# JuanTarrio/rebvo

Measured on NVIDIA H100. Metric: frames/sec @752x480 EuRoC replay (synthetic stand-in), detect+track+map; pose ATE vs reference in `parity`, higher is better.
Workload: dtype f32 scale space/detector + f64 tracker/EKF

## Files before the change

### include/rebvo_b200.h

```cpp
#ifndef REBVO_B200_H
#define REBVO_B200_H

#include <stdint.h>

#ifdef __cplusplus
extern "C" {
#endif

typedef struct rb_ctx rb_ctx;
typedef struct rb_map rb_map;
typedef struct rb_pipeline rb_pipeline;

enum rb_status {
    RB_OK = 0,
    RB_ERR_CUDA = -1,
    RB_ERR_ARG = -2,
    RB_ERR_NO_DEVICE = -3,
    RB_ERR_STATE = -4
};

typedef struct rb_keyline {
    int32_t p_inx;
    float m_m[2], u_m[2], n_m, score, c_p[2];
    int32_t _pad0;
// ... 72 lines not shown

int rb_map_create(rb_ctx *c, rb_map **out);
void rb_map_destroy(rb_map *m);
int rb_map_clone(const rb_map *src, rb_map **out);

int rb_map_upload_rgb(rb_map *m, const uint8_t *rgb);
int rb_map_upload_mono(rb_map *m, const uint8_t *mono);
int rb_map_upload_gray(rb_map *m, const float *gray);
int rb_map_dog_build(rb_map *m);
int rb_map_get_plane(rb_map *m, int which, float *out);
int rb_map_detect(rb_map *m, const rb_detect_params *p, double *tresh, int *l_kl_num, int *kn_out);
int rb_map_detect_ss(rb_map *m, rb_map *ss, const rb_detect_params *p, double *tresh, int *l_kl_num,
                     int *kn_out);
int rb_map_reestimate_thresh(rb_map *m, int knum, int nbins, float *out_thresh);
int rb_map_knum(rb_map *m, int *kn);
int rb_map_sync_host_keylines(rb_map *m, rb_keyline *dst, int capacity, int *kn);
int rb_map_load_keylines(rb_map *m, const rb_keyline *src, int kn, const int32_t *mask);
int rb_map_get_mask(rb_map *m, int32_t *out);

int rb_map_quantile(rb_map *m, double s_rho_min, double s_rho_max, double percentile, int nbins,
                    double *out);
int rb_map_build_field(rb_map *m, int radius, float min_mod);
int rb_map_get_field(rb_map *m, int32_t *out);
int rb_try_vel_rot(rb_map *fmap, rb_map *old, const double X[6], int reweight, int procjf,
                   double match_thresh, double s_rho_min, uint32_t match_num_thresh, double k_huber,
                   const double *res_in, double *res_out, double JtJ[36], double JtF[6], double *score);
int rb_minimizer_rv(rb_map *fmap, rb_map *old, double V[3], double W[3], double RVel[9], double RW0[9],
                    double match_thresh, int iter_max, int init_type, double reweight_distance,
                    double *rel_error, double *rel_error_score, double max_s_rho,
                    uint32_t match_num_thresh, int init_iter, double W_X[36], double *score);
// ... 69 lines not shown
```

### rebvo_b200/capi.py

```python
import ctypes as C
import os

import numpy as np

HERE = os.path.dirname(os.path.abspath(__file__))
LIB_PATH = os.environ.get("REBVO_B200_LIB") or os.path.join(HERE, "librebvo_b200.so")


class RbError(RuntimeError):
    pass


class Camera(C.Structure):
    _fields_ = [("w", C.c_int32), ("h", C.c_int32), ("ppx", C.c_float), ("ppy", C.c_float),
                ("zfx", C.c_float), ("zfy", C.c_float)]


class DetectParams(C.Structure):
    _fields_ = [("plane_fit_size", C.c_int32), ("pos_neg_thresh", C.c_double), ("dog_thresh", C.c_double),
                ("kl_max", C.c_int32), ("kl_ref", C.c_int32), ("gain", C.c_double),
                ("thresh_max", C.c_double), ("thresh_min", C.c_double)]


class Params(C.Structure):
# ... 36 lines not shown
KEYLINE = np.dtype({
    "names": ["p_inx", "m_m", "u_m", "n_m", "score", "c_p", "rho", "s_rho", "rho_nr", "s_rho_nr",
              "rho0", "s_rho0", "p_m", "p_m_0", "m_id", "m_id_f", "m_id_kf", "m_num", "m_m0", "n_m0",
              "p_id", "n_id", "net_id", "stereo_m_id", "stereo_rho", "stereo_s_rho"],
    "formats": ["i4", ("f4", 2), ("f4", 2), "f4", "f4", ("f4", 2), "f8", "f8", "f8", "f8", "f8", "f8",
                ("f4", 2), ("f4", 2), "i4", "i4", "i4", "i4", ("f4", 2), "f8", "i4", "i4", "i4", "i4",
                "f8", "f8"],
    "offsets": [0, 4, 12, 20, 24, 28, 40, 48, 56, 64, 72, 80, 88, 96, 104, 108, 112, 116, 120, 128,
                136, 140, 144, 148, 152, 160],
    "itemsize": 168})

SYMBOLS = ["rb_ctx_create", "rb_ctx_destroy", "rb_last_error", "rb_ctx_sync", "rb_ctx_box_plan",
           "rb_ctx_launch_count", "rb_map_create", "rb_map_destroy", "rb_map_clone", "rb_map_upload_rgb", "rb_map_upload_mono",
           "rb_map_upload_gray",
           "rb_map_dog_build", "rb_map_get_plane", "rb_map_detect", "rb_map_detect_ss", "rb_map_reestimate_thresh", "rb_map_knum",
           "rb_map_sync_host_keylines", "rb_map_load_keylines", "rb_map_get_mask", "rb_map_quantile",
           "rb_map_build_field", "rb_map_get_field", "rb_try_vel_rot", "rb_minimizer_rv", "rb_forward_match",
           "rb_map_rotate_keylines", "rb_directed_matching", "rb_map_regularize", "rb_map_ekf_update",
           "rb_map_rescale_opt", "rb_map_set_frame_count", "rb_pipeline_create", "rb_pipeline_destroy",
           "rb_pipeline_last_error", "rb_pipeline_push", "rb_pipeline_push_dev", "rb_pipeline_push_mono",
           "rb_pipeline_push_mono_dev", "rb_pipeline_reset",
           "rb_pipeline_map", "rb_pipeline_launch_count", "rb_pipeline_stage_ms", "rb_pipeline_stream",
           "rb_pipeline_event_record", "rb_pipeline_event_elapsed", "rb_pipeline_event_elapsed_between", "rb_pipeline_bench_pass",
           "rb_pipeline_set_imu", "rb_pipeline_set_mirror", "rb_pipeline_mirror", "rb_pipeline_set_undistort",
           "rb_pipeline_stage_profile",
           "rb_undistort_create", "rb_undistort_destroy", "rb_undistort_rgb", "rb_undistort_rgb_dev",
           "rb_try_vel", "rb_minimizer_v", "rb_ext_rot_vel", "rb_bias_correct", "rb_map_pack_net_keylines",
           "rb_nav_format_trajectory", "rb_nav_format_log", "rb_map_scale_space_path"]

_lib = None
# ... 176 lines not shown
    def detect(self, det, tresh, l_kl_num):
        t, l, kn = C.c_double(tresh), C.c_int(l_kl_num), C.c_int(0)
        self.ctx.check(self.L.rb_map_detect(self.h_, C.byref(det), C.byref(t), C.byref(l), C.byref(kn)))
        return kn.value, t.value, l.value

    def reestimate(self, knum, nbins):
        o = C.c_float(0)
        self.ctx.check(self.L.rb_map_reestimate_thresh(self.h_, knum, nbins, C.byref(o)))
        return o.value

    def knum(self):
        k = C.c_int(0)
        self.ctx.check(self.L.rb_map_knum(self.h_, C.byref(k)))
        return k.value

    def keylines(self):
        kn = self.knum()
        out = np.zeros(max(kn, 1), KEYLINE)
        k = C.c_int(0)
        self.ctx.check(self.L.rb_map_sync_host_keylines(self.h_, _p(out), len(out), C.byref(k)))
        return out[:kn]

    def scale_space_path(self):
        return int(self.L.rb_map_scale_space_path(self.h_))

    def pack_net(self, k_prof=1.0, capacity=None):
        cap = capacity if capacity is not None else max(self.knum(), 1)
        out = np.zeros((cap, 15), np.uint8)
        k = C.c_int(0)
        self.ctx.check(self.L.rb_map_pack_net_keylines(self.h_, C.c_double(k_prof), _p(out), cap, C.byref(k)))
# ... 255 lines not shown
```

### rebvo_b200/csrc/capi.cu

```cuda
#include <math.h>
#include <stdlib.h>
#include <new>

#include "common.cuh"
#include "tracker.cuh"

int rb_detect_upload_pinv(rb_ctx *c);

static void box_plan_one(double sigma, int box_n, int *box_d, double *sigma_r) {
    const double wideal = sqrt(12 * sigma * sigma / box_n + 1);
    int wl = (int)wideal;
    const int tmp = wl / 2;
    if (tmp * 2 == wl) wl--;
    const int m = (int)round((3 * box_n + 4 * box_n * wl + box_n * wl * wl - 12 * sigma * sigma) / (4 + 4 * wl));
    int i = 0;
    for (; i < m && i < box_n; i++) box_d[i] = wl;
    for (; i < box_n; i++) box_d[i] = wl + 2;
    *sigma_r = sqrt((m * wl * wl + (box_n - m) * (wl + 2.0) * (wl + 2.0) - box_n) / 12.0);
}

static void plane_fit_pinv(double pinv[3][25]) {
    const int ws = 2;
    double Phi[25][3];
    int k = 0;
// ... 491 lines not shown
    if ((r = read_state(m, &s))) return r;
    if (out_thresh) *out_thresh = s.retuned;
    return RB_OK;
}

extern "C" int rb_map_knum(rb_map *m, int *kn) {
    if (!m) return RB_ERR_ARG;
    RB_ENTER(m->c);
    MapState s;
    int r = read_state(m, &s);
    if (r) return r;
    *kn = s.kn;
    return RB_OK;
}

extern "C" int rb_map_scale_space_path(const rb_map *m) {
    if (!m || !m->ws.gray) return 0;
    return (m->ws.tma_row_ok ? 1 : 0) | (m->ws.tma_ok ? 2 : 0);
}

extern "C" int rb_map_sync_host_keylines(rb_map *m, rb_keyline *dst, int capacity, int *kn) {
    if (!m) return RB_ERR_ARG;
    RB_ENTER(m->c);
    rb_ctx *c = m->c;
    MapState s;
    int r = read_state(m, &s);
    if (r) return r;
    if (kn) *kn = s.kn;
    if (s.kn == 0) return RB_OK;
    if (!dst || capacity < s.kn) return RB_ERR_ARG;
// ... 53 lines not shown
```

### rebvo_b200/csrc/min_cluster.cuh

```cuda
#ifndef MC_T
#error "define MC_T and MC_NS before including min_cluster.cuh"
#endif
#undef MC_NW
#undef MC_MAXJ
#undef MC_NV
#define MC_NW (MC_T / 32)
#define MC_MAXJ (3584 / MC_T)
#define MC_NV (MC_MAXJ * MC_NW)

#ifndef MC_COMMON_PART
#define MC_COMMON_PART
#define MC_C 16
#define MC_GMAX 8
#define MC_PW 30
#define MC_XW 60
#ifndef MC_KPC_FAST
#define MC_KPC_FAST 1280
#endif
#define MC_SPIN_LIMIT (1ll << 29)
#define MC_BYTES_PER_KL 57

#ifdef RB_TVR_PROF
#define MC_STAMP(e, k) do { if (threadIdx.x == 0 && blockIdx.x < 16) g_tvr_prof[(blockIdx.x * 16 + (e)) * 16 + (k)] = clock64(); } while (0)
#else
// ... 454 lines not shown
    so3_exp(wz, RMf);
    sm.req[p][12] = RMf[0];
    sm.req[p][13] = RMf[1];
    sm.req[p][14] = RMf[3];
    sm.req[p][15] = RMf[4];
}

template <int XCHG>
__global__ void __cluster_dims__(MC_C, 1, 1) __launch_bounds__(MC_T, 1)
    k_minimizer_cluster(KLSoA old, const MapState *__restrict__ old_st, const unsigned long long *__restrict__ field,
                        const float4 *__restrict__ fpack, MapState *f_st, LMState *lm_out, int *abort_out, CamC cam,
                        McPlan plan, MinSetup su, FrameState *post_fs, FmBest *fm_best, int kpc_cap, ResPtrs gres,
                        unsigned long long *ll, MinCtl *ctl) {
    MC_STAMP(15, 0);
    const bool early = su.early_operands != 0 && su.a.match_num_thresh <= 255u;
    if (!early) {
        pdl_wait();
        pdl_launch();
    }
    MC_STAMP(15, 1);
    extern __shared__ __align__(16) unsigned char mc_dyn[];
    __shared__ McSmem sm;
    const int tid = threadIdx.x, lane = tid & 31, wid = tid >> 5;
    const int rank = (int)mc_cluster_rank();
    const int G = (int)(gridDim.x / MC_C), cl = (int)(blockIdx.x / MC_C);
    const bool first_cta = blockIdx.x == 0;
    const unsigned int seq0 = G > 1 ? __ldcg(&ctl->gen) : 0u;
    const int K0 = old_st->kn;
    if (K0 <= 0) {
        if (early) {
            pdl_wait();
            pdl_launch();
        }
        if (first_cta && tid == 0) {
// ... 45 lines not shown
        if (li < v.S) {
            const KlOp o = load_klop(old, v.base + li, cam);
            v.x0[li] = o.x0;
            v.y0[li] = o.y0;
            v.z0[li] = o.z0;
            v.s_rho[li] = o.s_rho;
            const unsigned int mn = (unsigned int)o.m_num;
            v.flag[li] = early ? (unsigned char)(mn < 255u ? mn : 255u) : (unsigned char)(mn < tc.mnt ? 1 : 0);
            v.res[0][li] = 0.0;
        } else {
            v.gres[0][v.base + li] = 0.0;
        }
    }
    if (early) {
        pdl_wait();
        pdl_launch();
        tc.s_rho_min = su.s_rho_from_state ? old_st->s_rho_q : su.max_s_rho;
        const unsigned int fc = su.fc_from_state ? f_st->frame_count : su.frame_count;
        tc.mnt = su.a.match_num_thresh < fc ? su.a.match_num_thresh : fc;
        const int ns = v.cnt < v.S ? v.cnt : v.S;
        for (int li = tid; li < ns; li += MC_T) v.flag[li] = (unsigned int)v.flag[li] < tc.mnt ? 1 : 0;
    }
    const bool fused = plan.merge_round >= 0;
    if (tid == 0) {
        sm.abort = su.debug_abort;
        lm_begin(sm.lm, old_st, f_st, su.VW, su.a, su.max_r, su.max_s_rho, su.s_rho_from_state, su.frame_count,
                 su.fc_from_state);
        if (fused) {
            for (int i = 0; i < 3; i++) {
                sm.lm.X[i] = sm.lm.Vel_in[i];
                sm.lm.X[3 + i] = sm.lm.W0_in[i];
// ... 17 lines not shown
    mc_cluster_sync();
    MC_STAMP(15, 2);

    for (int e = 0; e < plan.n; e++) {
        const int sa = plan.sa[e], sb = plan.sb[e];
        const bool two = sa != STEP_NONE;
        const bool RW = sb >= STEP_MAIN_FIRST;
        const bool PJ = !(sb == STEP_INIT_LAST_ZERO || sb == STEP_INIT_LAST_PRIOR);
        const int par = e & 1;
        const unsigned int nval = two ? 2 * MC_PW : MC_PW;
        const bool last = e == plan.n - 1;
        const bool merge = e == plan.merge_round;
        const bool next_two = !last && plan.sa[e + 1] != STEP_NONE;
        const int res_out_p[2] = {sm.req_res[0][1], sm.req_res[1][1]};
        MC_STAMP(e, 0);
        if (RW) mc_eval_pose<true, true>(sm, v, 0, old, tc, cam, field, fpack, last, tid, lane, wid);
        else if (PJ) mc_eval_pose<false, true>(sm, v, 0, old, tc, cam, field, fpack, last, tid, lane, wid);
        else mc_eval_pose<false, false>(sm, v, 0, old, tc, cam, field, fpack, last, tid, lane, wid);
        if (two) {
            if (PJ) mc_eval_pose<false, true>(sm, v, 1, old, tc, cam, field, fpack, false, tid, lane, wid);
            else mc_eval_pose<false, false>(sm, v, 1, old, tc, cam, field, fpack, false, tid, lane, wid);
        }
        __syncthreads();
        MC_STAMP(e, 1);
        const unsigned int seq = seq0 + 1u + (unsigned int)e;
        if (XCHG && tid == 0) mc_mbar_expect_tx(&sm.mbar[par], nval * MC_C * 8u);
        if (wid < 2 && (wid == 0 || two)) {
            const int p = wid;
            double t = lane < MC_PW ? sm.xout[p * MC_PW + lane] : 0.0;
            if (G > 1) {
// ... 194 lines not shown
```

### rebvo_b200/csrc/pipeline.cu

```cuda
#include <math.h>
#include <stdlib.h>
#include <new>

#include "common.cuh"
#include "lm.cuh"
#include "tracker.cuh"
#include "frame.cuh"

int rb_map_alloc(rb_ctx *c, rb_map **out, bool with_ws);

#define RB_NMAPS 3

#ifdef RB_TVR_PROF
__device__ unsigned long long g_trace[8192];
__device__ unsigned int g_trace_n;
__global__ void k_trace_mark(int tag) {
    unsigned long long t;
    asm volatile("mov.u64 %0, %globaltimer;" : "=l"(t));
    const unsigned int k = atomicAdd(&g_trace_n, 1u);
    if (k < 8192) g_trace[k] = ((unsigned long long)tag << 56) | (t & 0x00FFFFFFFFFFFFFFull);
}
extern "C" int rb_debug_fetch_trace(unsigned long long *out, unsigned int *n) {
    cudaMemcpyFromSymbol(n, g_trace_n, sizeof(unsigned int));
    cudaMemcpyFromSymbol(out, g_trace, sizeof(unsigned long long) * 8192);
// ... 7 lines not shown

struct ImuFlow;
struct rb_pipeline {
    rb_ctx *c;
    ImuFlow *imu;
    rb_params p;
    int max_batch;
    DogWS ws;
    rb_map *maps[RB_NMAPS];
    cudaStream_t det_stream;
    cudaEvent_t ev_dog, *ev_det, *ev_trk;
    bool overlap;
    bool q_fold;
    int ss_sub;
    bool map_fused;
    cudaStream_t resc_stream;
    cudaEvent_t ev_rfork, ev_rjoin;
    bool resc_open;
    cudaStream_t copy_stream;
    cudaEvent_t *ev_copy;
    const void **rgb_src_dev;
    const void **rgb_src_pin;
    int sub;
    DetChain *chain;
    FrameState *fs;
    rb_nav *nav_dev;
    rb_nav *nav_pin;
    int *abort_pin;
    uint8_t *rgb_pin;
    long long n_pushed;
// ... 170 lines not shown
    const char *ng = getenv("REBVO_B200_NO_GRAPH");
    pl->use_graph = !(ng && ng[0] == '1');
    const char *sp = getenv("REBVO_B200_STAGE_PROF");
    pl->prof_on = sp && sp[0] == '1';
    if (pl->prof_on) {
        pl->use_graph = false;
        pl->pcap = max_batch * 12 + 8;
        pl->pev = new (std::nothrow) cudaEvent_t[pl->pcap];
        pl->ptag = new (std::nothrow) int[pl->pcap];
        if (!pl->pev || !pl->ptag) return RB_ERR_ARG;
        for (int i = 0; i < pl->pcap; i++) RB_CUDA(cudaEventCreate(&pl->pev[i]));
    }
    {
        const char *mf = getenv("REBVO_B200_MAP_FUSED");
        pl->map_fused = mf ? atoi(mf) != 0 : false;
        const char *ov = getenv("REBVO_B200_OVERLAP");
        pl->overlap = !(ov && ov[0] == '0') && !pl->prof_on;
        pl->q_fold = getenv("REBVO_B200_Q_FOLD") && atoi(getenv("REBVO_B200_Q_FOLD")) != 0 && p->QCutOffNumBins >= 1 &&
                     p->QCutOffNumBins <= 128;
        pl->ss_sub = getenv("REBVO_B200_SS_SUB") ? atoi(getenv("REBVO_B200_SS_SUB")) : 0;
        if (pl->ss_sub < 4) pl->ss_sub = 0;
        pl->ev_det = new (std::nothrow) cudaEvent_t[max_batch];
        pl->ev_trk = new (std::nothrow) cudaEvent_t[max_batch];
        if (!pl->ev_det || !pl->ev_trk) return RB_ERR_ARG;
        memset(pl->ev_det, 0, sizeof(cudaEvent_t) * max_batch);
        memset(pl->ev_trk, 0, sizeof(cudaEvent_t) * max_batch);
        RB_CUDA(cudaStreamCreateWithFlags(&pl->det_stream, cudaStreamNonBlocking));
        RB_CUDA(cudaStreamCreateWithFlags(&pl->copy_stream, cudaStreamNonBlocking));
        const char *sb = getenv("REBVO_B200_SUB");
        pl->sub = sb ? atoi(sb) : 8;
// ... 156 lines not shown
    a.reweight_distance = p.ReweigthDistance;
    a.match_num_thresh = p.MatchNumThresh;
    RB_TRACE(c->stream, 2);
    bool folded = false;
    c->min_early = !pl->q_fold && (getenv("REBVO_B200_MIN_EARLY") ? atoi(getenv("REBVO_B200_MIN_EARLY")) != 0 : true);
    r = rb_minimizer_enqueue(c, neu, old, pl->fs->VW, &a, 0.0, true, 0, true, pl->fs, &folded);
    c->min_early = false;
    if (r) return r;
    RB_TRACE(c->stream, 3);
    prof_mark(pl, ST_MINIM);
    if (!folded) {
        k_frame_post_min<<<1, 1, 0, c->stream>>>(pl->fs, neu->ts);
        RB_LAUNCH_CHECK();
        if ((r = rb_forward_match_argmax_enqueue(c, old, neu))) return r;
    }
    if ((r = resc_join(pl))) return r;
    if ((r = rb_forward_match_apply_enqueue(c, old, neu, pl->fs->R0))) return r;
    RB_TRACE(c->stream, 11);
    prof_mark(pl, ST_FWD_ROT);
    if ((r = rb_directed_matching_enqueue(c, neu, old, &pl->fs->dm, p.MatchThreshModule, p.MatchThreshAngle,
                                          (double)p.SearchRange, p.LocationUncertaintyMatch, &pl->fs->do_match)))
        return r;
    RB_TRACE(c->stream, 4);
    prof_mark(pl, ST_DMATCH);
    const bool side = pl->resc_stream != nullptr && pl->mirror_on != 1;
    if (!pl->map_fused)
        if ((r = rb_regularize_ekf_enqueue(c, neu, p.RegularizeThresh, pl->fs, p.MatchThreshold, pl->fs->V,
                                           p.ReshapeQAbsolute, p.LocationUncertainty, &pl->fs->do_map,
                                           side ? old->st : nullptr, side ? nav_slot : nullptr, fa)))
            return r;
    RB_TRACE(c->stream, 9);
    prof_mark(pl, ST_REG_EKF);
    if (side) {
        cudaStream_t main_stream = c->stream;
        RB_CUDA(cudaEventRecord(pl->ev_rfork, main_stream));
        RB_CUDA(cudaStreamWaitEvent(pl->resc_stream, pl->ev_rfork, 0));
        c->stream = pl->resc_stream;
        r = rb_rescale_enqueue(c, neu, RB_RHO_MAX, 1, 0, &neu->st->do_map, nav_slot);
        c->stream = main_stream;
        if (r) return r;
        RB_CUDA(cudaEventRecord(pl->ev_rjoin, pl->resc_stream));
        pl->resc_open = true;
        RB_TRACE(c->stream, 5);
        return RB_OK;
    }
// ... 380 lines not shown
```

### rebvo_b200/csrc/tracker.cu

```cuda
#include "tracker.cuh"
#include "lm.cuh"
#include "frame.cuh"

#define TVR_T 256
#define RES_SENTINEL 0x7FF8DEADBEEF0001ull

#ifdef RB_TVR_PROF
__device__ long long g_tvr_prof[256 * 16];
#define TVR_STAMP(k) do { if (threadIdx.x == 0) g_tvr_prof[blockIdx.x * 16 + (k)] = clock64(); } while (0)
__device__ __forceinline__ long long tvr_gtime() {
    long long t;
    asm volatile("mov.u64 %0, %globaltimer;" : "=l"(t));
    return t;
}
#define TVR_GSTAMP(k) do { if (threadIdx.x == 0) g_tvr_prof[blockIdx.x * 16 + (k)] = tvr_gtime(); } while (0)
extern "C" int rb_debug_fetch(long long *out) {
    return (int)cudaMemcpyFromSymbol(out, g_tvr_prof, sizeof(long long) * 256 * 16);
}
#else
#define TVR_STAMP(k) do { } while (0)
#define TVR_GSTAMP(k) do { } while (0)
#endif

struct CamC {
// ... 1220 lines not shown
}

int rb_try_vel_rot_enqueue(rb_ctx *c, rb_map *fmap, rb_map *old, const double *X_dev, int reweight, int procjf,
                           double match_thresh, double s_rho_min, unsigned int mnt, unsigned int fc,
                           double k_huber) {
    if (fmap->field_radius <= 0) return RB_ERR_STATE;
    k_lm_single<<<1, 1, 0, c->stream>>>(fmap->ts, X_dev, 0, 1, (double)fmap->field_radius, match_thresh, s_rho_min,
                                        mnt, fc, k_huber);
    RB_LAUNCH_CHECK();
    if (reweight && procjf) return launch_eval<true, true>(c, fmap, old, STEP_NONE);
    if (reweight) return launch_eval<true, false>(c, fmap, old, STEP_NONE);
    if (procjf) return launch_eval<false, true>(c, fmap, old, STEP_NONE);
    return launch_eval<false, false>(c, fmap, old, STEP_NONE);
}

__device__ __forceinline__ void d_rotate_vals(const KLSoA &kl, int i, const double (&R)[9], double zf, float2 pm, double rho,
                                              double s_rho, float2 m) {
    const double v0 = (double)pm.x / zf, v1 = (double)pm.y / zf, v2 = 1;
    double q0 = 0, q1 = 0, q2 = 0;
    q0 = q0 + R[0] * v0; q0 = q0 + R[1] * v1; q0 = q0 + R[2] * v2;
    q1 = q1 + R[3] * v0; q1 = q1 + R[4] * v1; q1 = q1 + R[5] * v2;
    q2 = q2 + R[6] * v0; q2 = q2 + R[7] * v1; q2 = q2 + R[8] * v2;
    if (fabs(q2) > 0) {
        kl.p_m[i] = make_float2((float)(q0 / q2 * zf), (float)(q1 / q2 * zf));
        kl.rho[i] = rho / q2;
        kl.s_rho[i] = s_rho / q2;
    }
    const double m0 = (double)m.x, m1 = (double)m.y;
    double r0 = 0, r1 = 0;
    r0 = r0 + R[0] * m0; r0 = r0 + R[1] * m1; r0 = r0 + R[2] * 0.0;
    r1 = r1 + R[3] * m0; r1 = r1 + R[4] * m1; r1 = r1 + R[5] * 0.0;
    const float2 mr = make_float2((float)r0, (float)r1);
    kl.m_m[i] = mr;
    float4 p = kl.pack[2 * i];
    p.x = mr.x;
    p.y = mr.y;
    kl.pack[2 * i] = p;
}
__device__ __forceinline__ void d_rotate(const KLSoA &kl, int i, const double *__restrict__ Rp, double zf) {
    double R[9];
#pragma unroll
    for (int k = 0; k < 9; k++) R[k] = Rp[k];
    d_rotate_vals(kl, i, R, zf, kl.p_m[i], kl.rho[i], kl.s_rho[i], kl.m_m[i]);
}
__global__ void __launch_bounds__(256) k_rotate(KLSoA kl, const MapState *st, const double *__restrict__ Rp,
                                                double zf) {
    pdl_wait();
// ... 76 lines not shown
        k_set_int<<<1, 1, 0, c->stream>>>(&neu->st->fwd_match, 0);
        RB_LAUNCH_CHECK();
    }
    int r;
    if ((r = rb_forward_match_init_enqueue(c, neu))) return r;
    if ((r = rb_forward_match_argmax_enqueue(c, old, neu))) return r;
    return rb_forward_match_apply_enqueue(c, old, neu, nullptr);
}

int rb_rotate_enqueue(rb_ctx *c, rb_map *m, const double *R_dev) {
    RB_KLAUNCH(k_rotate, rb_div_up(c->kcap, 256), 256, 0, m->kl, (const MapState *)m->st, R_dev, c->zfm);
    return RB_OK;
}

#define DM_G 4
__global__ void __launch_bounds__(128) k_directed_match(KLSoA neu, MapState *nst, KLSoA old,
                                                        const int *__restrict__ omask, const DMatchArgs *__restrict__ ap,
                                                        CamC cam, double min_thr_mod, double cang_min_edge,
                                                        double max_radius, double loc_unc, const int *enable) {
    pdl_wait();
    pdl_launch();
    if (enable && !*enable) return;
    const int gi = blockIdx.x * blockDim.x + threadIdx.x;
    const int i = gi / DM_G, g = gi % DM_G, lane = threadIdx.x & 31;
    bool got = false;
    int jm = -1;
    {
        const bool valid = i < nst->kn;
        const int ic = valid ? i : 0;
        const double zf = cam.zfm;
        const double *BR = ap->BackRot, *Vel = ap->Vel, *RV = ap->RVel;
        const float2 kpm = neu.p_m[ic];
        const double krho = neu.rho[ic], ks_rho = neu.s_rho[ic];
        const float2 km = neu.m_m[ic];
        const float kn_m = neu.n_m[ic];
        const double a0 = (double)kpm.x, a1 = (double)kpm.y, a2 = zf;
        double p30 = 0, p31 = 0, p32 = 0;
        p30 = p30 + BR[0] * a0; p30 = p30 + BR[1] * a1; p30 = p30 + BR[2] * a2;
        p31 = p31 + BR[3] * a0; p31 = p31 + BR[4] * a1; p31 = p31 + BR[5] * a2;
        p32 = p32 + BR[6] * a0; p32 = p32 + BR[7] * a1; p32 = p32 + BR[8] * a2;
        const float pmx = (float)(p30 * zf / p32), pmy = (float)(p31 * zf / p32);
        const double k_rho = krho * zf / p32;
        const float pi0x = pmx + cam.ppx, pi0y = pmy + cam.ppy;
        double t_x = -(Vel[0] * zf - Vel[2] * (double)pmx);
        double t_y = -(Vel[1] * zf - Vel[2] * (double)pmy);
        double norm_t = sqrt(t_x * t_x + t_y * t_y);
        const double D0 = zf, D1 = zf, D2 = (double)(-pmx - pmy);
        double r0 = 0, r1 = 0, r2 = 0;
        r0 = r0 + D0 * RV[0]; r0 = r0 + D1 * RV[3]; r0 = r0 + D2 * RV[6];
        r1 = r1 + D0 * RV[1]; r1 = r1 + D1 * RV[4]; r1 = r1 + D2 * RV[7];
// ... 35 lines not shown
            tn -= 1;
        }
        bool active = valid;
        while (true) {
            int j_hit = -1;
            if (active && t_i < t_steps) {
                const double t = dir ? tp : tn;
                const bool inside = dir ? !(t > dq_max) : !(t < dq_min);
                if (inside) {
                    const float fx = (float)(t_x * t + (double)pi0x), fy = (float)(t_y * t + (double)pi0y);
                    const int xi = (int)roundf(fx), yi = (int)roundf(fy);
                    if (!(xi >= cam.w || yi >= cam.h || xi < 0 || yi < 0)) {
                        const int j = omask[(size_t)yi * cam.w + xi];
                        if (j >= 0) {
                            const double norm_m0 = (double)old.n_m[j];
                            const float2 om = old.m_m[j];
                            const double cang = (double)(om.x * km.x + om.y * km.y) / (norm_m0 * norm_m);
                            if (!(cang < cang_min_edge || fabs(norm_m0 / norm_m - 1) > min_thr_mod)) {
                                const double s_rho = old.s_rho[j], rho = old.rho[j];
                                const double v_rho_dr = (loc_unc * loc_unc + s_rho * s_rho * norm_t * norm_t + sigma2_t * rho * rho);
                                const double e = t - norm_t * rho;
                                if (!(e * e > v_rho_dr)) j_hit = j;
                            }
                        }
                    }
                }
            }
            const unsigned int bal = __ballot_sync(0xffffffffu, j_hit >= 0);
            const unsigned int grp = (bal >> (lane & ~(DM_G - 1))) & ((1u << DM_G) - 1u);
            const int src = grp ? (lane & ~(DM_G - 1)) + __ffs(grp) - 1 : lane;
            const int jw = __shfl_sync(0xffffffffu, j_hit, src);
            if (grp) {
                jm = jw;
                active = false;
            }
#pragma unroll
            for (int k = 0; k < DM_G / 2; k++) {
                tp += 1;
                tn -= 1;
            }
            t_i += DM_G / 2;
            if (!__any_sync(0xffffffffu, active && t_i < t_steps)) break;
        }
        if (g != 0) jm = -1;
        if (jm >= 0) {
            neu.rho[i] = old.rho[jm];
            neu.s_rho[i] = old.s_rho[jm];
            neu.m_id[i] = jm;
            neu.m_num[i] = old.m_num[jm] + 1;
            neu.p_m_0[i] = old.p_m[jm];
            neu.m_m0[i] = old.m_m[jm];
            neu.n_m0[i] = (double)old.n_m[jm];
            got = true;
        }
    }
    const unsigned int bal = __ballot_sync(0xffffffffu, got);
    if ((threadIdx.x & 31) == 0 && bal) atomicAdd(&nst->nmatch, __popc(bal));
}

int rb_directed_matching_enqueue(rb_ctx *c, rb_map *neu, rb_map *old, const DMatchArgs *args_dev, double min_thr_mod,
                                 double min_thr_ang, double max_radius, double loc_uncertainty, const int *enable_dev) {
    const double cang_min_edge = cos(min_thr_ang * M_PI / 180.0);
    if (!c->counters_preset) {
        k_set_int<<<1, 1, 0, c->stream>>>(&neu->st->nmatch, 0);
        RB_LAUNCH_CHECK();
    }
    RB_KLAUNCH(k_directed_match, rb_div_up(c->kcap * DM_G, 128), 128, 0, neu->kl, neu->st, old->kl, old->mask, args_dev,
               make_cam(c), min_thr_mod, cang_min_edge, max_radius, loc_uncertainty, enable_dev);
    return RB_OK;
}

__device__ __forceinline__ bool d_reg_a(const KLSoA &kl, int i, double *__restrict__ r, double *__restrict__ s,
                                        unsigned char *__restrict__ set, double thresh) {
    bool did = false;
    unsigned char sv = 0;
    const int ni = kl.n_id[i], pi = kl.p_id[i];
    if (ni >= 0 && pi >= 0) {
        const double krho = kl.rho[i], ks = kl.s_rho[i];
        const double nrho = kl.rho[ni], ns = kl.s_rho[ni];
        const double prho = kl.rho[pi], ps = kl.s_rho[pi];
        const double d = nrho - prho;
        if (!(d * d > ns * ns + ps * ps)) {
            const float2 nm = kl.m_m[ni], pmv = kl.m_m[pi];
            const float nnm = kl.n_m[ni], pnm = kl.n_m[pi];
            double alpha = (double)((nm.x * pmv.x + nm.y * pmv.y) / (nnm * pnm));
            if (!(alpha - thresh < 0)) {
                alpha = (alpha - thresh) / (1 - thresh);
                alpha /= fabs(nrho - prho) / (ns + ps) + 1;
                const double wr = 1 / (ks * ks);
                const double wrn = alpha / (ns * ns);
                const double wrp = alpha / (ps * ps);
                r[i] = (krho * wr + nrho * wrn + prho * wrp) / (wr + wrn + wrp);
                s[i] = (ks * wr + ns * wrn + ps * wrp) / (wr + wrn + wrp);
                sv = 1;
                did = true;
            }
        }
    }
    set[i] = sv;
    return did;
}
__global__ void __launch_bounds__(256) k_regularize_a(KLSoA kl, MapState *st, double *__restrict__ r,
                                                      double *__restrict__ s, unsigned char *__restrict__ set,
                                                      double thresh, const int *enable) {
    if (enable && !*enable) return;
    const int i = blockIdx.x * blockDim.x + threadIdx.x;
    const bool did = i < st->kn ? d_reg_a(kl, i, r, s, set, thresh) : false;
    const unsigned int bal = __ballot_sync(0xffffffffu, did);
    if ((threadIdx.x & 31) == 0 && bal) atomicAdd(&st->reg_num, __popc(bal));
}
__global__ void __launch_bounds__(256) k_regularize_b(KLSoA kl, const MapState *st, const double *__restrict__ r,
                                                      const double *__restrict__ s,
                                                      const unsigned char *__restrict__ set, const int *enable) {
    if (enable && !*enable) return;
// ... 110 lines not shown
        rho = kl.rho[i];
        s_rho = kl.s_rho[i];
    }
    if (kl.m_id[i] < 0) return;
    d_ekf(kl, i, rho, s_rho, velp, zf, q_abs, loc_unc);
}
int rb_regularize_ekf_enqueue(rb_ctx *c, rb_map *m, double thresh, FrameState *fs, int match_threshold,
                              const double *vel_dev, double q_abs, double loc_unc, const int *do_map_dev,
                              const MapState *ost, rb_nav *nav, const FrameArgs *fa) {
    TrackState &t = m->ts_host;
    const int nb = rb_div_up(c->kcap, 256);
    RB_KLAUNCH(k_regularize_a_gate, nb, 256, 0, m->kl, m->st, t.reg_r, t.reg_s, t.reg_set, thresh, fs, match_threshold);
    RB_KLAUNCH(k_regb_ekf, nb, 256, 0, m->kl, (const MapState *)m->st, (const double *)t.reg_r, (const double *)t.reg_s,
               (const unsigned char *)t.reg_set, vel_dev, c->zfm, q_abs, loc_unc, do_map_dev, fs, ost,
               (const LMState *)&m->ts->lm, nav, fa);
    return RB_OK;
}



#include <cooperative_groups.h>
namespace cg = cooperative_groups;
#define MU_T 512
#define MU_C 16
#define MU_QBINS 128
#define MU_KJ 2

struct MapUpdArgs {
    int do_reg, do_ekf, do_rescale, re_escale, gate_post_match;
    double reg_thresh;
// ... 303 lines not shown
```

### rebvo_b200/csrc/tracker.cuh

```cuda
#pragma once
#include "common.cuh"

enum LMStep {
    STEP_NONE = 0,
    STEP_INIT_FIRST_ZERO,
    STEP_INIT_ITER_ZERO,
    STEP_INIT_LAST_ZERO,
    STEP_INIT_FIRST_PRIOR,
    STEP_INIT_ITER_PRIOR,
    STEP_INIT_LAST_PRIOR,
    STEP_MAIN_FIRST,
    STEP_MAIN_ITER,
    STEP_MAIN_LAST
};

struct MinCtl {
    unsigned int gen;
    int abort;
};

struct __align__(16) FmBest {
    unsigned long long key;
    long long idx;
};
// ... 27 lines not shown
int rb_forward_match_init_enqueue(rb_ctx *c, rb_map *neu);
int rb_forward_match_argmax_enqueue(rb_ctx *c, rb_map *old, rb_map *neu);
int rb_forward_match_apply_enqueue(rb_ctx *c, rb_map *old, rb_map *neu, const double *R_dev);
int rb_forward_match_enqueue(rb_ctx *c, rb_map *old, rb_map *neu);
int rb_rotate_enqueue(rb_ctx *c, rb_map *m, const double *R_dev);
struct DMatchArgs {
    double Vel[3];
    double RVel[9];
    double BackRot[9];
};
int rb_directed_matching_enqueue(rb_ctx *c, rb_map *neu, rb_map *old, const DMatchArgs *args_dev,
                                 double min_thr_mod, double min_thr_ang, double max_radius,
                                 double loc_uncertainty, const int *enable_dev);
int rb_regularize_enqueue(rb_ctx *c, rb_map *m, double thresh, const int *enable_dev);
struct rb_nav;
int rb_regularize_ekf_enqueue(rb_ctx *c, rb_map *m, double thresh, FrameState *fs, int match_threshold,
                              const double *vel_dev, double q_abs, double loc_unc, const int *do_map_dev,
                              const MapState *ost = nullptr, rb_nav *nav = nullptr, const FrameArgs *fa = nullptr);
int rb_map_update_enqueue(rb_ctx *c, rb_map *m, double reg_thresh, const double *vel_dev, double q_abs,
                          double loc_unc, double s_rho_min, unsigned int match_num_min, int re_escale,
                          FrameState *fs, int match_threshold, const MapState *ost, rb_nav *nav,
                          const FrameArgs *fa, bool fused = false, const rb_quantile_fold *qf = nullptr);
int rb_ekf_enqueue(rb_ctx *c, rb_map *m, const double *vel_dev, double q_abs, double loc_unc,
                   const int *enable_dev);
int rb_rescale_enqueue(rb_ctx *c, rb_map *m, double s_rho_min, unsigned int match_num_min, int re_escale,
                       const int *enable_dev, rb_nav *kp_nav = nullptr);
int rb_read_map_state(rb_map *m, MapState *host);
```

Baseline: 7170.

## Chain forward-match apply, directed matching and regularize+EKF into two fused kernels

Adds a default-on map_chain path. The forward-match apply and directed matching are merged into a single k_match kernel that rotates old keylines on the fly, writing regularization inputs to scratch. The regularize and EKF passes are merged into one k_reg_ekf kernel that also rotates the old map in place. The minimizer's PDL launch trigger is moved to the last step so the dependent kernel starts earlier. This cuts kernel launches and global round-trips per frame, at the cost of redundant rotation math inside the search loop and a possible numeric divergence.

New measurement: 7544, median of 6. 5.2% higher.

```diff
diff --git a/include/rebvo_b200.h b/include/rebvo_b200.h
--- a/include/rebvo_b200.h
+++ b/include/rebvo_b200.h
@@ -110,6 +110,7 @@
                      int *kn_out);
 int rb_map_reestimate_thresh(rb_map *m, int knum, int nbins, float *out_thresh);
 int rb_map_knum(rb_map *m, int *kn);
+int rb_map_counters(rb_map *m, int out[3]);
 int rb_map_sync_host_keylines(rb_map *m, rb_keyline *dst, int capacity, int *kn);
 int rb_map_load_keylines(rb_map *m, const rb_keyline *src, int kn, const int32_t *mask);
 int rb_map_get_mask(rb_map *m, int32_t *out);
diff --git a/rebvo_b200/capi.py b/rebvo_b200/capi.py
--- a/rebvo_b200/capi.py
+++ b/rebvo_b200/capi.py
@@ -74,6 +74,7 @@
            "rb_ctx_launch_count", "rb_map_create", "rb_map_destroy", "rb_map_clone", "rb_map_upload_rgb", "rb_map_upload_mono",
            "rb_map_upload_gray",
            "rb_map_dog_build", "rb_map_get_plane", "rb_map_detect", "rb_map_detect_ss", "rb_map_reestimate_thresh", "rb_map_knum",
+           "rb_map_counters",
            "rb_map_sync_host_keylines", "rb_map_load_keylines", "rb_map_get_mask", "rb_map_quantile",
            "rb_map_build_field", "rb_map_get_field", "rb_try_vel_rot", "rb_minimizer_rv", "rb_forward_match",
            "rb_map_rotate_keylines", "rb_directed_matching", "rb_map_regularize", "rb_map_ekf_update",
@@ -280,6 +281,11 @@
         self.ctx.check(self.L.rb_map_knum(self.h_, C.byref(k)))
         return k.value
 
+    def counters(self):
+        out = (C.c_int * 3)()
+        self.ctx.check(self.L.rb_map_counters(self.h_, out))
+        return tuple(out)
+
     def keylines(self):
         kn = self.knum()
         out = np.zeros(max(kn, 1), KEYLINE)
diff --git a/rebvo_b200/csrc/capi.cu b/rebvo_b200/csrc/capi.cu
--- a/rebvo_b200/csrc/capi.cu
+++ b/rebvo_b200/csrc/capi.cu
@@ -529,6 +529,18 @@
     return RB_OK;
 }
 
+extern "C" int rb_map_counters(rb_map *m, int out[3]) {
+    if (!m || !out) return RB_ERR_ARG;
+    RB_ENTER(m->c);
+    MapState s;
+    int r = read_state(m, &s);
+    if (r) return r;
+    out[0] = s.fwd_match;
+    out[1] = s.nmatch;
+    out[2] = s.reg_num;
+    return RB_OK;
+}
+
 extern "C" int rb_map_scale_space_path(const rb_map *m) {
     if (!m || !m->ws.gray) return 0;
     return (m->ws.tma_row_ok ? 1 : 0) | (m->ws.tma_ok ? 2 : 0);
diff --git a/rebvo_b200/csrc/min_cluster.cuh b/rebvo_b200/csrc/min_cluster.cuh
--- a/rebvo_b200/csrc/min_cluster.cuh
+++ b/rebvo_b200/csrc/min_cluster.cuh
@@ -492,10 +492,7 @@
                         unsigned long long *ll, MinCtl *ctl) {
     MC_STAMP(15, 0);
     const bool early = su.early_operands != 0 && su.a.match_num_thresh <= 255u;
-    if (!early) {
-        pdl_wait();
-        pdl_launch();
-    }
+    if (!early) pdl_wait();
     MC_STAMP(15, 1);
     extern __shared__ __align__(16) unsigned char mc_dyn[];
     __shared__ McSmem sm;
@@ -571,7 +568,6 @@
     }
     if (early) {
         pdl_wait();
-        pdl_launch();
         tc.s_rho_min = su.s_rho_from_state ? old_st->s_rho_q : su.max_s_rho;
         const unsigned int fc = su.fc_from_state ? f_st->frame_count : su.frame_count;
         tc.mnt = su.a.match_num_thresh < fc ? su.a.match_num_thresh : fc;
@@ -619,6 +615,7 @@
         const bool next_two = !last && plan.sa[e + 1] != STEP_NONE;
         const int res_out_p[2] = {sm.req_res[0][1], sm.req_res[1][1]};
         MC_STAMP(e, 0);
+        if (last) pdl_launch();
         if (RW) mc_eval_pose<true, true>(sm, v, 0, old, tc, cam, field, fpack, last, tid, lane, wid);
         else if (PJ) mc_eval_pose<false, true>(sm, v, 0, old, tc, cam, field, fpack, last, tid, lane, wid);
         else mc_eval_pose<false, false>(sm, v, 0, old, tc, cam, field, fpack, last, tid, lane, wid);
diff --git a/rebvo_b200/csrc/pipeline.cu b/rebvo_b200/csrc/pipeline.cu
--- a/rebvo_b200/csrc/pipeline.cu
+++ b/rebvo_b200/csrc/pipeline.cu
@@ -45,6 +45,7 @@
     bool q_fold;
     int ss_sub;
     bool map_fused;
+    bool map_chain;
     cudaStream_t resc_stream;
     cudaEvent_t ev_rfork, ev_rjoin;
     bool resc_open;
@@ -245,6 +246,8 @@
     {
         const char *mf = getenv("REBVO_B200_MAP_FUSED");
         pl->map_fused = mf ? atoi(mf) != 0 : false;
+        const char *mc = getenv("REBVO_B200_MAP_CHAIN");
+        pl->map_chain = !(mc && atoi(mc) == 0) && !pl->map_fused;
         const char *ov = getenv("REBVO_B200_OVERLAP");
         pl->overlap = !(ov && ov[0] == '0') && !pl->prof_on;
         pl->q_fold = getenv("REBVO_B200_Q_FOLD") && atoi(getenv("REBVO_B200_Q_FOLD")) != 0 && p->QCutOffNumBins >= 1 &&
@@ -431,21 +434,34 @@
         RB_LAUNCH_CHECK();
         if ((r = rb_forward_match_argmax_enqueue(c, old, neu))) return r;
     }
-    if ((r = resc_join(pl))) return r;
-    if ((r = rb_forward_match_apply_enqueue(c, old, neu, pl->fs->R0))) return r;
-    RB_TRACE(c->stream, 11);
-    prof_mark(pl, ST_FWD_ROT);
-    if ((r = rb_directed_matching_enqueue(c, neu, old, &pl->fs->dm, p.MatchThreshModule, p.MatchThreshAngle,
-                                          (double)p.SearchRange, p.LocationUncertaintyMatch, &pl->fs->do_match)))
-        return r;
-    RB_TRACE(c->stream, 4);
-    prof_mark(pl, ST_DMATCH);
     const bool side = pl->resc_stream != nullptr && pl->mirror_on != 1;
-    if (!pl->map_fused)
-        if ((r = rb_regularize_ekf_enqueue(c, neu, p.RegularizeThresh, pl->fs, p.MatchThreshold, pl->fs->V,
-                                           p.ReshapeQAbsolute, p.LocationUncertainty, &pl->fs->do_map,
-                                           side ? old->st : nullptr, side ? nav_slot : nullptr, fa)))
+    if (pl->map_chain) {
+        if ((r = resc_join(pl))) return r;
+        prof_mark(pl, ST_FWD_ROT);
+        if ((r = rb_match_enqueue(c, neu, old, &pl->fs->dm, pl->fs->R0, p.MatchThreshModule, p.MatchThreshAngle,
+                                  (double)p.SearchRange, p.LocationUncertaintyMatch, &pl->fs->do_match)))
             return r;
+        RB_TRACE(c->stream, 4);
+        prof_mark(pl, ST_DMATCH);
+        if ((r = rb_reg_ekf_enqueue(c, neu, old, p.RegularizeThresh, pl->fs, p.MatchThreshold, p.ReshapeQAbsolute,
+                                    p.LocationUncertainty, pl->fs->R0, side ? nav_slot : nullptr, fa)))
+            return r;
+    } else {
+        if ((r = resc_join(pl))) return r;
+        if ((r = rb_forward_match_apply_enqueue(c, old, neu, pl->fs->R0))) return r;
+        RB_TRACE(c->stream, 11);
+        prof_mark(pl, ST_FWD_ROT);
+        if ((r = rb_directed_matching_enqueue(c, neu, old, &pl->fs->dm, p.MatchThreshModule, p.MatchThreshAngle,
+                                              (double)p.SearchRange, p.LocationUncertaintyMatch, &pl->fs->do_match)))
+            return r;
+        RB_TRACE(c->stream, 4);
+        prof_mark(pl, ST_DMATCH);
+        if (!pl->map_fused)
+            if ((r = rb_regularize_ekf_enqueue(c, neu, p.RegularizeThresh, pl->fs, p.MatchThreshold, pl->fs->V,
+                                               p.ReshapeQAbsolute, p.LocationUncertainty, &pl->fs->do_map,
+                                               side ? old->st : nullptr, side ? nav_slot : nullptr, fa)))
+                return r;
+    }
     RB_TRACE(c->stream, 9);
     prof_mark(pl, ST_REG_EKF);
     if (side) {
diff --git a/rebvo_b200/csrc/tracker.cu b/rebvo_b200/csrc/tracker.cu
--- a/rebvo_b200/csrc/tracker.cu
+++ b/rebvo_b200/csrc/tracker.cu
@@ -1258,23 +1258,38 @@
     return launch_eval<false, false>(c, fmap, old, STEP_NONE);
 }
 
-__device__ __forceinline__ void d_rotate_vals(const KLSoA &kl, int i, const double (&R)[9], double zf, float2 pm, double rho,
-                                              double s_rho, float2 m) {
+struct RotPt {
+    float2 pm;
+    double rho, s_rho;
+};
+__device__ __forceinline__ RotPt d_rot_pt(const double (&R)[9], double zf, float2 pm, double rho, double s_rho) {
     const double v0 = (double)pm.x / zf, v1 = (double)pm.y / zf, v2 = 1;
     double q0 = 0, q1 = 0, q2 = 0;
     q0 = q0 + R[0] * v0; q0 = q0 + R[1] * v1; q0 = q0 + R[2] * v2;
     q1 = q1 + R[3] * v0; q1 = q1 + R[4] * v1; q1 = q1 + R[5] * v2;
     q2 = q2 + R[6] * v0; q2 = q2 + R[7] * v1; q2 = q2 + R[8] * v2;
+    RotPt o = {pm, rho, s_rho};
     if (fabs(q2) > 0) {
-        kl.p_m[i] = make_float2((float)(q0 / q2 * zf), (float)(q1 / q2 * zf));
-        kl.rho[i] = rho / q2;
-        kl.s_rho[i] = s_rho / q2;
-    }
+        o.pm = make_float2((float)(q0 / q2 * zf), (float)(q1 / q2 * zf));
+        o.rho = rho / q2;
+        o.s_rho = s_rho / q2;
+    }
+    return o;
+}
+__device__ __forceinline__ float2 d_rot_m(const double (&R)[9], float2 m) {
     const double m0 = (double)m.x, m1 = (double)m.y;
     double r0 = 0, r1 = 0;
     r0 = r0 + R[0] * m0; r0 = r0 + R[1] * m1; r0 = r0 + R[2] * 0.0;
     r1 = r1 + R[3] * m0; r1 = r1 + R[4] * m1; r1 = r1 + R[5] * 0.0;
-    const float2 mr = make_float2((float)r0, (float)r1);
+    return make_float2((float)r0, (float)r1);
+}
+__device__ __forceinline__ void d_rotate_vals(const KLSoA &kl, int i, const double (&R)[9], double zf, float2 pm, double rho,
+                                              double s_rho, float2 m) {
+    const RotPt pt = d_rot_pt(R, zf, pm, rho, s_rho);
+    kl.p_m[i] = pt.pm;
+    kl.rho[i] = pt.rho;
+    kl.s_rho[i] = pt.s_rho;
+    const float2 mr = d_rot_m(R, m);
     kl.m_m[i] = mr;
     float4 p = kl.pack[2 * i];
     p.x = mr.x;
@@ -1381,26 +1396,17 @@
 }
 
 #define DM_G 4
-__global__ void __launch_bounds__(128) k_directed_match(KLSoA neu, MapState *nst, KLSoA old,
-                                                        const int *__restrict__ omask, const DMatchArgs *__restrict__ ap,
-                                                        CamC cam, double min_thr_mod, double cang_min_edge,
-                                                        double max_radius, double loc_unc, const int *enable) {
-    pdl_wait();
-    pdl_launch();
-    if (enable && !*enable) return;
-    const int gi = blockIdx.x * blockDim.x + threadIdx.x;
-    const int i = gi / DM_G, g = gi % DM_G, lane = threadIdx.x & 31;
-    bool got = false;
+template <bool ROT>
+__device__ __forceinline__ int d_dm_search(const KLSoA &old, const int *__restrict__ omask,
+                                           const DMatchArgs *__restrict__ ap, const CamC &cam, double min_thr_mod,
+                                           double cang_min_edge, double max_radius, double loc_unc, bool valid, int g,
+                                           float2 kpm, double krho, double ks_rho, float2 km, float kn_m,
+                                           const double (&R)[9]) {
+    const int lane = threadIdx.x & 31;
     int jm = -1;
     {
-        const bool valid = i < nst->kn;
-        const int ic = valid ? i : 0;
         const double zf = cam.zfm;
         const double *BR = ap->BackRot, *Vel = ap->Vel, *RV = ap->RVel;
-        const float2 kpm = neu.p_m[ic];
-        const double krho = neu.rho[ic], ks_rho = neu.s_rho[ic];
-        const float2 km = neu.m_m[ic];
-        const float kn_m = neu.n_m[ic];
         const double a0 = (double)kpm.x, a1 = (double)kpm.y, a2 = zf;
         double p30 = 0, p31 = 0, p32 = 0;
         p30 = p30 + BR[0] * a0; p30 = p30 + BR[1] * a1; p30 = p30 + BR[2] * a2;
@@ -1466,10 +1472,15 @@
                         const int j = omask[(size_t)yi * cam.w + xi];
                         if (j >= 0) {
                             const double norm_m0 = (double)old.n_m[j];
-                            const float2 om = old.m_m[j];
+                            const float2 om = ROT ? d_rot_m(R, old.m_m[j]) : old.m_m[j];
                             const double cang = (double)(om.x * km.x + om.y * km.y) / (norm_m0 * norm_m);
                             if (!(cang < cang_min_edge || fabs(norm_m0 / norm_m - 1) > min_thr_mod)) {
-                                const double s_rho = old.s_rho[j], rho = old.rho[j];
+                                double s_rho = old.s_rho[j], rho = old.rho[j];
+                                if (ROT) {
+                                    const RotPt pt = d_rot_pt(R, zf, old.p_m[j], rho, s_rho);
+                                    rho = pt.rho;
+                                    s_rho = pt.s_rho;
+                                }
                                 const double v_rho_dr = (loc_unc * loc_unc + s_rho * s_rho * norm_t * norm_t + sigma2_t * rho * rho);
                                 const double e = t - norm_t * rho;
                                 if (!(e * e > v_rho_dr)) j_hit = j;
@@ -1494,20 +1505,100 @@
             t_i += DM_G / 2;
             if (!__any_sync(0xffffffffu, active && t_i < t_steps)) break;
         }
-        if (g != 0) jm = -1;
+    }
+    return jm;
+}
+__global__ void __launch_bounds__(128) k_directed_match(KLSoA neu, MapState *nst, KLSoA old,
+                                                        const int *__restrict__ omask, const DMatchArgs *__restrict__ ap,
+                                                        CamC cam, double min_thr_mod, double cang_min_edge,
+                                                        double max_radius, double loc_unc, const int *enable) {
+    pdl_wait();
+    pdl_launch();
+    if (enable && !*enable) return;
+    const int gi = blockIdx.x * blockDim.x + threadIdx.x;
+    const int i = gi / DM_G, g = gi % DM_G;
+    const bool valid = i < nst->kn;
+    const int ic = valid ? i : 0;
+    const double R[9] = {};
+    int jm = d_dm_search<false>(old, omask, ap, cam, min_thr_mod, cang_min_edge, max_radius, loc_unc, valid, g,
+                                neu.p_m[ic], neu.rho[ic], neu.s_rho[ic], neu.m_m[ic], neu.n_m[ic], R);
+    bool got = false;
+    if (g != 0) jm = -1;
+    if (jm >= 0) {
+        neu.rho[i] = old.rho[jm];
+        neu.s_rho[i] = old.s_rho[jm];
+        neu.m_id[i] = jm;
+        neu.m_num[i] = old.m_num[jm] + 1;
+        neu.p_m_0[i] = old.p_m[jm];
+        neu.m_m0[i] = old.m_m[jm];
+        neu.n_m0[i] = (double)old.n_m[jm];
+        got = true;
+    }
+    const unsigned int bal = __ballot_sync(0xffffffffu, got);
+    if ((threadIdx.x & 31) == 0 && bal) atomicAdd(&nst->nmatch, __popc(bal));
+}
+
+__global__ void __launch_bounds__(128) k_match(KLSoA neu, MapState *nst, KLSoA old, const int *__restrict__ omask,
+                                               const FmBest *best, const DMatchArgs *__restrict__ ap,
+                                               const double *__restrict__ Rp, double *__restrict__ reg_r,
+                                               double *__restrict__ reg_s, CamC cam, double min_thr_mod,
+                                               double cang_min_edge, double max_radius, double loc_unc,
+                                               const int *__restrict__ do_match) {
+    pdl_wait();
+    pdl_launch();
+    if ((int)(blockIdx.x * (blockDim.x / DM_G)) >= nst->kn) return;
+    const int gi = blockIdx.x * blockDim.x + threadIdx.x;
+    const int i = gi / DM_G, g = gi % DM_G;
+    const bool valid = i < nst->kn;
+    const int ic = valid ? i : 0;
+    const longlong2 b = __ldcg(reinterpret_cast<const longlong2 *>(best + ic));
+    const float2 kpm = neu.p_m[ic], km = neu.m_m[ic];
+    const float kn_m = neu.n_m[ic];
+    double R[9];
+#pragma unroll
+    for (int k = 0; k < 9; k++) R[k] = Rp[k];
+    const int fw = valid ? (int)b.y : -1;
+    double krho, ks_rho;
+    if (fw >= 0) {
+        krho = old.rho[fw];
+        ks_rho = old.s_rho[fw];
+    } else {
+        krho = neu.rho[ic];
+        ks_rho = neu.s_rho[ic];
+    }
+    int jm = -1;
+    if (*do_match)
+        jm = d_dm_search<true>(old, omask, ap, cam, min_thr_mod, cang_min_edge, max_radius, loc_unc, valid, g, kpm, krho,
+                               ks_rho, km, kn_m, R);
+    bool got = false;
+    if (valid && g == 0) {
+        double rho = krho, s_rho = ks_rho;
         if (jm >= 0) {
-            neu.rho[i] = old.rho[jm];
-            neu.s_rho[i] = old.s_rho[jm];
+            const RotPt pt = d_rot_pt(R, cam.zfm, old.p_m[jm], old.rho[jm], old.s_rho[jm]);
+            rho = pt.rho;
+            s_rho = pt.s_rho;
             neu.m_id[i] = jm;
             neu.m_num[i] = old.m_num[jm] + 1;
-            neu.p_m_0[i] = old.p_m[jm];
-            neu.m_m0[i] = old.m_m[jm];
+            neu.p_m_0[i] = pt.pm;
+            neu.m_m0[i] = d_rot_m(R, old.m_m[jm]);
             neu.n_m0[i] = (double)old.n_m[jm];
             got = true;
-        }
+        } else if (fw >= 0) {
+            neu.m_id[i] = fw;
+            neu.m_num[i] = old.m_num[fw] + 1;
+            neu.p_m_0[i] = old.p_m[fw];
+            neu.m_m0[i] = old.m_m[fw];
+            neu.n_m0[i] = (double)old.n_m[fw];
+        }
+        reg_r[i] = rho;
+        reg_s[i] = s_rho;
     }
     const unsigned int bal = __ballot_sync(0xffffffffu, got);
-    if ((threadIdx.x & 31) == 0 && bal) atomicAdd(&nst->nmatch, __popc(bal));
+    const unsigned int fbal = __ballot_sync(0xffffffffu, valid && g == 0 && fw >= 0);
+    if ((threadIdx.x & 31) == 0) {
+        if (bal) atomicAdd(&nst->nmatch, __popc(bal));
+        if (fbal) atomicAdd(&nst->fwd_match, __popc(fbal));
+    }
 }
 
 int rb_directed_matching_enqueue(rb_ctx *c, rb_map *neu, rb_map *old, const DMatchArgs *args_dev, double min_thr_mod,
@@ -1521,16 +1612,25 @@
                make_cam(c), min_thr_mod, cang_min_edge, max_radius, loc_uncertainty, enable_dev);
     return RB_OK;
 }
-
-__device__ __forceinline__ bool d_reg_a(const KLSoA &kl, int i, double *__restrict__ r, double *__restrict__ s,
-                                        unsigned char *__restrict__ set, double thresh) {
+int rb_match_enqueue(rb_ctx *c, rb_map *neu, rb_map *old, const DMatchArgs *args_dev, const double *R_dev,
+                     double min_thr_mod, double min_thr_ang, double max_radius, double loc_uncertainty,
+                     const int *do_match_dev) {
+    const double cang_min_edge = cos(min_thr_ang * M_PI / 180.0);
+    const TrackState &t = neu->ts_host;
+    RB_KLAUNCH(k_match, rb_div_up(c->kcap * DM_G, 128), 128, 0, neu->kl, neu->st, old->kl, (const int *)old->mask,
+               (const FmBest *)t.fm_best, args_dev, R_dev, t.reg_r, t.reg_s, make_cam(c), min_thr_mod, cang_min_edge,
+               max_radius, loc_uncertainty, do_match_dev);
+    return RB_OK;
+}
+
+__device__ __forceinline__ bool d_reg_vals(const KLSoA &kl, int i, const double *rho, const double *s_rho, double thresh,
+                                           double &r_out, double &s_out) {
     bool did = false;
-    unsigned char sv = 0;
     const int ni = kl.n_id[i], pi = kl.p_id[i];
     if (ni >= 0 && pi >= 0) {
-        const double krho = kl.rho[i], ks = kl.s_rho[i];
-        const double nrho = kl.rho[ni], ns = kl.s_rho[ni];
-        const double prho = kl.rho[pi], ps = kl.s_rho[pi];
+        const double krho = rho[i], ks = s_rho[i];
+        const double nrho = rho[ni], ns = s_rho[ni];
+        const double prho = rho[pi], ps = s_rho[pi];
         const double d = nrho - prho;
         if (!(d * d > ns * ns + ps * ps)) {
             const float2 nm = kl.m_m[ni], pmv = kl.m_m[pi];
@@ -1542,14 +1642,18 @@
                 const double wr = 1 / (ks * ks);
                 const double wrn = alpha / (ns * ns);
                 const double wrp = alpha / (ps * ps);
-                r[i] = (krho * wr + nrho * wrn + prho * wrp) / (wr + wrn + wrp);
-                s[i] = (ks * wr + ns * wrn + ps * wrp) / (wr + wrn + wrp);
-                sv = 1;
+                r_out = (krho * wr + nrho * wrn + prho * wrp) / (wr + wrn + wrp);
+                s_out = (ks * wr + ns * wrn + ps * wrp) / (wr + wrn + wrp);
                 did = true;
             }
         }
     }
-    set[i] = sv;
+    return did;
+}
+__device__ __forceinline__ bool d_reg_a(const KLSoA &kl, int i, double *__restrict__ r, double *__restrict__ s,
+                                        unsigned char *__restrict__ set, double thresh) {
+    const bool did = d_reg_vals(kl, i, kl.rho, kl.s_rho, thresh, r[i], s[i]);
+    set[i] = did ? 1 : 0;
     return did;
 }
 __global__ void __launch_bounds__(256) k_regularize_a(KLSoA kl, MapState *st, double *__restrict__ r,
@@ -1690,6 +1794,45 @@
     RB_KLAUNCH(k_regb_ekf, nb, 256, 0, m->kl, (const MapState *)m->st, (const double *)t.reg_r, (const double *)t.reg_s,
                (const unsigned char *)t.reg_set, vel_dev, c->zfm, q_abs, loc_unc, do_map_dev, fs, ost,
                (const LMState *)&m->ts->lm, nav, fa);
+    return RB_OK;
+}
+
+__global__ void __launch_bounds__(256) k_reg_ekf(KLSoA kl, MapState *st, const double *__restrict__ r,
+                                                 const double *__restrict__ s, double thresh, FrameState *fs,
+                                                 int match_threshold, double zf, double q_abs, double loc_unc, KLSoA old,
+                                                 const MapState *ost, const double *__restrict__ Rp, const LMState *lm,
+                                                 rb_nav *nav, const FrameArgs *fa) {
+    pdl_wait();
+    pdl_launch();
+    if (blockIdx.x == gridDim.x - 1 && threadIdx.x == 0) {
+        d_frame_post_match(fs, st, match_threshold);
+        st->do_map = fs->do_map;
+        if (nav) d_frame_finish(fs, st, ost, lm->score, nav, fa, false);
+        else d_frame_pose(fs);
+    }
+    const int i = blockIdx.x * blockDim.x + threadIdx.x;
+    if (i < ost->kn) d_rotate(old, i, Rp, zf);
+    const bool en = fs->do_match && st->nmatch >= match_threshold;
+    bool did = false;
+    if (i < st->kn) {
+        double rho = r[i], s_rho = s[i];
+        if (en) did = d_reg_vals(kl, i, r, s, thresh, rho, s_rho);
+        if (en && kl.m_id[i] >= 0) {
+            d_ekf(kl, i, rho, s_rho, fs->V, zf, q_abs, loc_unc);
+        } else {
+            kl.rho[i] = rho;
+            kl.s_rho[i] = s_rho;
+        }
+    }
+    const unsigned int bal = __ballot_sync(0xffffffffu, did);
+    if ((threadIdx.x & 31) == 0 && bal) atomicAdd(&st->reg_num, __popc(bal));
+}
+int rb_reg_ekf_enqueue(rb_ctx *c, rb_map *m, rb_map *old, double thresh, FrameState *fs, int match_threshold,
+                       double q_abs, double loc_unc, const double *R_dev, rb_nav *nav, const FrameArgs *fa) {
+    const TrackState &t = m->ts_host;
+    RB_KLAUNCH(k_reg_ekf, rb_div_up(c->kcap, 256), 256, 0, m->kl, m->st, (const double *)t.reg_r,
+               (const double *)t.reg_s, thresh, fs, match_threshold, c->zfm, q_abs, loc_unc, old->kl,
+               (const MapState *)old->st, R_dev, (const LMState *)&m->ts->lm, nav, fa);
     return RB_OK;
 }
 
diff --git a/rebvo_b200/csrc/tracker.cuh b/rebvo_b200/csrc/tracker.cuh
--- a/rebvo_b200/csrc/tracker.cuh
+++ b/rebvo_b200/csrc/tracker.cuh
@@ -65,6 +65,11 @@
                                  double loc_uncertainty, const int *enable_dev);
 int rb_regularize_enqueue(rb_ctx *c, rb_map *m, double thresh, const int *enable_dev);
 struct rb_nav;
+int rb_match_enqueue(rb_ctx *c, rb_map *neu, rb_map *old, const DMatchArgs *args_dev, const double *R_dev,
+                     double min_thr_mod, double min_thr_ang, double max_radius, double loc_uncertainty,
+                     const int *do_match_dev);
+int rb_reg_ekf_enqueue(rb_ctx *c, rb_map *m, rb_map *old, double thresh, FrameState *fs, int match_threshold,
+                       double q_abs, double loc_unc, const double *R_dev, rb_nav *nav, const FrameArgs *fa);
 int rb_regularize_ekf_enqueue(rb_ctx *c, rb_map *m, double thresh, FrameState *fs, int match_threshold,
                               const double *vel_dev, double q_abs, double loc_unc, const int *do_map_dev,
                               const MapState *ost = nullptr, rb_nav *nav = nullptr, const FrameArgs *fa = nullptr);
```
